# cyoq/onitama-alphazero

Hardware: AMD Instinct MI355X
Metric: MCTS node-expansions/sec/GPU @400 sims; self-play games/sec at 1/2/4/8 GPU (higher is better)
Workload: dtype fp32 (fp16x3 split)

## Files before the change

### onitama-alphazero_amd/csrc/oaz_engine.cpp

```cpp
#include <hip/hip_runtime.h>

#include <math.h>
#include <stddef.h>
#include <time.h>
#include <stdarg.h>
#include <stdio.h>
#include <stdlib.h>
#include <string.h>

#include <mutex>
#include <string>
#include <algorithm>
#include <vector>

#include "../../include/onitama_az.h"
#include "oaz_device.h"
#include "oaz_host.h"
#include "oaz_kernels.h"
#include "oaz_pack.h"
#include "oaz_weights_layout.h"

using namespace oaz;

static_assert(offsetof(oaz_config, search_time_ns) == 104 && offsetof(oaz_config, reuse_visits) == 116 &&
// ... 276 lines not shown
    if (!launch_reflect_samples) return oaz_set_err(OAZ_ERR_STATE, "reflect_samples: built without its kernel");
    RulesCtx* R = nullptr;
    std::unique_lock<std::mutex> lk;
    if (int rc = rules_begin(&R, lk)) return rc;
    hipStream_t st = R->stream;
    if (int rc = R->e.reserve(n)) return rc;
    if (int rc = R->f.reserve(n)) return rc;
    HIP_TRY(hipMemcpyAsync(R->e, in, n * sizeof(oaz_sample), hipMemcpyHostToDevice, st));
    HIP_TRY(launch_reflect_samples(R->e, n, R->f, st));
    HIP_TRY(hipMemcpyAsync(out, R->f, n * sizeof(oaz_sample), hipMemcpyDeviceToHost, st));
    HIP_TRY(hipStreamSynchronize(st));
    return 0;
}

constexpr int kMaxParts = 4;

enum LaunchKind { K_SELECT, K_NN, K_EXPAND, K_FINALIZE, K_NOISE, K_COMPACT, K_BACKUP_SELECT, K_COUNT };

struct TimedLaunch {
    LaunchKind kind;
    Event a, b;
    uint32_t samples;
};

struct LastSearch {
    uint32_t G = 0;
    uint32_t sims = 0;
    bool on_device = false;
    std::vector<uint32_t> per_game;
};
// ... 9 lines not shown
    uint32_t noise_chunk = 16;
    uint32_t G = 0, cap = 0, pathcap = 0, hcap = 0, out_cap = 0;
    int32_t sims_cap = 0;
    DevBuf<oaz_node> nodes;
    DevBuf<uint32_t> n_nodes, path, depth, leaf;
    DevBuf<oaz_state> leaf_state;
    DevBuf<uint64_t> stats, stats_sum;
    DevBuf<double> sqrt_tab;
    DevBuf<float> policy, value;
    DevBuf<uint8_t> need;
    DevBuf<uint32_t> slot, bcnt;
    DevBuf<oaz_state> cstate;
    DevBuf<float> weights;
    bool have_weights = false;
    DevBuf<unsigned long long> nn_fallback;
    DevBuf<oaz_state> s_roots;
    DevBuf<oaz_move> s_move;
    DevBuf<float> s_pi, s_rootv, s_rootp;
    uint32_t search_calls = 0;
    LastSearch last;
    DevBuf<uint64_t> deadline;
    DevBuf<uint32_t> sims_run;
    int wall_khz = 0;
    double t_search0 = 0.0;
    DevBuf<uint32_t> s_ply;
    DevBuf<oaz_state> root;
    DevBuf<uint32_t> ply, seq;
    DevBuf<uint64_t> game_id;
    DevBuf<uint8_t> active;
    DevBuf<oaz_sample> hist, out;
// ... 240 lines not shown
        for (auto& ev : e->ev_consumed[i])
            if (ev.create()) return OAZ_ERR_HIP;
    }
    if (hipDeviceGetAttribute(&e->cus, hipDeviceAttributeMultiprocessorCount, e->device) != hipSuccess || e->cus < 1)
        e->cus = 256;
    if (hipDeviceGetAttribute(&e->wall_khz, hipDeviceAttributeWallClockRate, e->device) != hipSuccess) e->wall_khz = 0;
    const size_t G = e->G;
    e->noise_chunk = noise_chunk_for(e);
    if (e->nodes.alloc(G * e->cap) || e->n_nodes.alloc(G) || e->path.alloc(G * e->pathcap) || e->depth.alloc(G) ||
        e->leaf.alloc(G) || e->leaf_state.alloc(G) || e->stats.alloc(G * GS_COUNT) || e->stats_sum.alloc(GS_COUNT) ||
        e->sqrt_tab.alloc((size_t)tree_visits_cap(cfg) + 2) || e->policy.alloc(G * 50) || e->value.alloc(G) || e->need.alloc(G) ||
        e->slot.alloc(G) || e->cstate.alloc(G + 16) || e->bcnt.alloc((size_t)buckets_of((uint32_t)G) + kMaxParts) ||
        e->weights.alloc(nn_device_floats(cfg->blocks, cfg->precision)) || e->s_roots.alloc(G) || e->s_move.alloc(G) ||
        e->s_pi.alloc(G * 50) || e->s_rootv.alloc(G) || e->s_rootp.alloc(G * 50) || e->s_ply.alloc(G) ||
        e->root.alloc(G) || e->ply.alloc(G) || e->seq.alloc(G) || e->game_id.alloc(G) || e->active.alloc(G) ||
        e->hist.alloc(G * e->hcap) || e->out.alloc(e->out_cap) || e->out_count.alloc(1) || e->nn_fallback.alloc(1) ||
        e->deadline.alloc(1) || e->sims_run.alloc(G) || e->fin.alloc(G) || e->fin_pos.alloc(G) ||
        (cfg->train_noise && e->noise.alloc(2 * (size_t)e->noise_chunk * G * kNoiseStride)))
        return OAZ_ERR_HIP;
    if (cfg->reuse_visits > 0 &&
        (e->adv_moves.alloc(G) || e->adv_codes.alloc(G) || e->adv_kept.alloc(G) || e->reuse_cnt.alloc(4)))
        return OAZ_ERR_HIP;
    if (cfg->temperature_plies > 0 && e->temp_cnt.alloc(2)) return OAZ_ERR_HIP;
    if (const size_t L = cfg->leaf_batch) {
        if (e->par_path.alloc(G * L * e->pathcap) || e->par_depth.alloc(G * L) || e->par_leaf.alloc(G * L) ||
            e->par_state.alloc(G * kMaxLeafBatch) || e->par_policy.alloc(G * kMaxLeafBatch * 50) ||
            e->par_value.alloc(G * kMaxLeafBatch) || e->par_stats.alloc(G * 3))
            return OAZ_ERR_HIP;
    }
    std::vector<double> tab((size_t)tree_visits_cap(cfg) + 2);
    for (size_t i = 0; i < tab.size(); ++i) tab[i] = sqrt((double)i);
    hipStream_t s0 = e->stream;
    HIP_TRY(hipMemcpyAsync(e->sqrt_tab, tab.data(), tab.size() * sizeof(double), hipMemcpyHostToDevice, s0));
    HIP_TRY(hipMemsetAsync(e->stats, 0, G * GS_COUNT * sizeof(uint64_t), s0));
    HIP_TRY(hipMemsetAsync(e->out_count, 0, sizeof(unsigned long long), s0));
    HIP_TRY(hipMemsetAsync(e->nn_fallback, 0, sizeof(unsigned long long), s0));
    HIP_TRY(hipMemsetAsync(e->active, 0, G, s0));
    HIP_TRY(hipMemsetAsync(e->need, 0, G, s0));
    HIP_TRY(hipMemsetAsync(e->slot, 0, G * sizeof(uint32_t), s0));
    HIP_TRY(hipMemsetAsync(e->cstate, 0, (G + 16) * sizeof(oaz_state), s0));
    if (e->reuse_cnt) HIP_TRY(hipMemsetAsync(e->reuse_cnt, 0, 4 * sizeof(uint64_t), s0));
    if (e->temp_cnt) HIP_TRY(hipMemsetAsync(e->temp_cnt, 0, 2 * sizeof(uint64_t), s0));
    if (e->par_state) {
        HIP_TRY(hipMemsetAsync(e->par_state, 0, G * kMaxLeafBatch * sizeof(oaz_state), s0));
        HIP_TRY(hipMemsetAsync(e->par_stats, 0, G * 3 * sizeof(uint64_t), s0));
    }
    HIP_TRY(hipStreamSynchronize(s0));
    if (cfg->evaluator == OAZ_EVAL_NN) {
        std::vector<float> w(oaz_weight_count(cfg->blocks, 64, 21));
        if (int rc = oaz_random_weights(0, cfg->blocks, w.data(), w.size())) return rc;
        if (int rc = oaz_load_weights(e, w.data(), w.size())) return rc;
// ... 135 lines not shown

extern "C" int oaz_kernel_times_get(oaz_engine* e, oaz_kernel_times* out) {
    if (!e || !out) return oaz_set_err(OAZ_ERR_ARG, "kernel_times: null");
    if (int rc = resolve_timing(e)) return rc;
    *out = e->times;
    return 0;
}

extern "C" int oaz_kernel_times_reset(oaz_engine* e) {
    if (!e) return oaz_set_err(OAZ_ERR_ARG, "kernel_times_reset: null");
    if (int rc = resolve_timing(e)) return rc;
    memset(&e->times, 0, sizeof(e->times));
    return 0;
}

static NNView nn_view(const oaz_engine* e, const TileMap* tm) {
    NNView w;
    w.blob = e->weights;
    w.blocks = e->cfg.blocks;
    w.precision = e->cfg.precision;
    w.x6_variant = 0;
#if OAZ_AB
    if (const char* xv = getenv("OAZ_NN_X6_V")) w.x6_variant = atoi(xv);
#endif
    w.blob_x6 = e->cfg.precision == OAZ_FP32_SPLIT16 ? e->weights + nn_packed_floats(e->cfg.blocks, OAZ_FP32_SPLIT16)
                                                     : nullptr;
    w.fallback = e->nn_fallback;
    w.tm = tm ? *tm : TileMap{nullptr, 0, 0};
    w.small_max = e->cus;
#if OAZ_AB
    if (const char* v = getenv("OAZ_NN_SMALL_MAX")) w.small_max = atoi(v);
#endif
    return w;
}

static int evaluate(oaz_engine* e, const oaz_state* d_states, uint32_t B, float* d_pol, float* d_val,
                    hipStream_t st = nullptr, const TileMap* tm = nullptr) {
    if (!st) st = e->stream;
    const uint32_t counted = tm ? 0u : B;
    if (e->cfg.evaluator == OAZ_EVAL_HASH)
        return timed(e, K_NN, counted, [&] { return launch_hash_eval(d_states, (int)B, d_pol, d_val, st); }, st);
    const NNView w = nn_view(e, tm);
    return timed(e, K_NN, counted, [&] { return launch_nn_forward(w, d_states, (int)B, d_pol, d_val, st); }, st);
}

extern "C" int oaz_nn_fallbacks(oaz_engine* e, uint64_t* tiles) {
    if (!e || !tiles) return oaz_set_err(OAZ_ERR_ARG, "nn_fallbacks: null");
    OAZ_ON_DEVICE(e->device);
    unsigned long long n = 0;
    HIP_TRY(hipMemcpyAsync(&n, e->nn_fallback, sizeof(n), hipMemcpyDeviceToHost, e->stream));
    HIP_TRY(hipStreamSynchronize(e->stream));
    *tiles = (uint64_t)n;
    return 0;
}

extern "C" int oaz_nn_forward(oaz_engine* e, const oaz_state* s, int B, float* policy, float* value) {
    if (!e || !s || B < 0) return oaz_set_err(OAZ_ERR_ARG, "nn_forward: bad arguments");
// ... 298 lines not shown
                if (int rc = backup(pc.fast)) return rc;
                for (int h = 0; h < P.n; ++h) P.part[h].active = pc.fullm + P.part[h].g0;
            }
            if (int rc = sim_step(e, S, P, ring, s, &spent)) return rc;
        }
        if (int rc = ring.release(c)) return rc;
    }
    if (int rc = backup(pc.fullm)) return rc;
    return P.join();
}

static int run_sims(oaz_engine* e, const TreeView& t, const oaz_state* roots, const uint8_t* active,
                    const uint64_t* gids, const uint32_t* plies, bool kept_trees = false, const PlyCap* pc = nullptr) {
    const bool budget = e->cfg.search_time_ns > 0, noise = e->cfg.train_noise && e->noise;
    const SearchPath path = pc ? PATH_STEPS : search_path(e, t.G, noise, kept_trees);
    const NNView w = nn_view(e, nullptr);
    Search S{t, roots, active, gids, plies, search_params(e), (uint32_t)e->cfg.sims, noise,
             e->cfg.evaluator == OAZ_EVAL_HASH ? nullptr : &w, budget ? e->deadline.get() : nullptr,
             budget ? e->sims_run.get() : nullptr};
    if (!pc && !compact_leaves(e, t.G)) {
        S.t.need = nullptr;
        S.t.slot = nullptr;
    }
    e->last = LastSearch{t.G};
    int rc = path == PATH_STEPS ? 0 : arm_device_budget(e, t.G);
    if (!rc)
        rc = pc                 ? run_capped(e, S, *pc)
             : path == PATH_PAR ? search_par(e, S)
             : path == PATH_LAT ? search_lat(e, S)
                                : run_chunks(e, S, path == PATH_GRP);
    if (rc) {
// ... 393 lines not shown
```

### onitama-alphazero_amd/csrc/oaz_kernels.h

```cpp
#pragma once

#include <hip/hip_runtime.h>
#include <stdint.h>

#include "../../include/onitama_az.h"
#include "oaz_device.h"
#include "oaz_nn_layout.h"

namespace oaz {

enum GameStat {
    GS_SIMS = 0,
    GS_EXPANSIONS,
    GS_CHILDREN,
    GS_TERMINAL,
    GS_DEPTH,
    GS_STUCK,
    GS_MAXNODES,
    GS_MOVES,
    GS_FINISHED,
    GS_CUT,
    GS_RED,
    GS_BLUE,
    GS_PASSES,
// ... 58 lines not shown
    const uint32_t* bcnt;
    int32_t nb;
    int32_t cap;
};
inline int32_t buckets_of(uint32_t G) { return (int32_t)((G + kBucket - 1) >> kBucketShift); }

struct NNView {
    const float* blob;
    int32_t blocks;
    int32_t precision;
    int32_t x6_variant;
    const float* blob_x6;
    unsigned long long* fallback;
    TileMap tm;
    int32_t small_max;
};

hipError_t launch_movegen(const oaz_state* s, int n, uint32_t* masks, oaz_move* moves,
                          uint8_t* counts, hipStream_t st);
hipError_t launch_step(oaz_state* s, const oaz_move* mv, int n, uint8_t* results, hipStream_t st);
hipError_t launch_current_state(const oaz_state* s, int n, uint8_t* results, hipStream_t st);
hipError_t launch_encode(const oaz_state* s, int n, float* planes, hipStream_t st);
__attribute__((weak)) hipError_t launch_reflect_samples(const oaz_sample* in, size_t n, oaz_sample* out, hipStream_t st);

hipError_t launch_nn_forward(const NNView& w, const oaz_state* s, int B, float* policy,
                             float* value, hipStream_t st);
hipError_t launch_hash_eval(const oaz_state* s, int B, float* policy, float* value, hipStream_t st);
hipError_t launch_eval_compact(const TreeView& t, hipStream_t st);

hipError_t launch_tree_reset(const TreeView& t, hipStream_t st);
constexpr int kNoiseStride = 2 * OAZ_MAX_MOVES;
hipError_t launch_select(const TreeView& t, const oaz_state* roots, const uint8_t* active,
                         const noise_t* noise , SearchParams p, hipStream_t st);
hipError_t launch_root_noise(const oaz_state* roots, const uint8_t* active, const uint64_t* game_id,
                             const uint32_t* ply, SearchParams p, uint32_t G, uint32_t sim0, uint32_t nsims,
                             noise_t* out , hipStream_t st);
hipError_t launch_expand_backup(const TreeView& t, const oaz_state* roots, const uint8_t* active,
                                const float* policy, const float* value, hipStream_t st);
hipError_t launch_backup_select(const TreeView& t, const oaz_state* roots, const uint8_t* active, const float* policy,
                                const float* value, const noise_t* noise, SearchParams p, hipStream_t st);
hipError_t launch_search_finalize(const TreeView& t, const oaz_state* roots, oaz_move* out_move,
// ... 45 lines not shown
```

### onitama-alphazero_amd/csrc/oaz_kernels.hip

```cpp
#include <hip/hip_runtime.h>
#include <stdlib.h>

#include <utility>

#include "oaz_device.h"
#include "oaz_kernels.h"

namespace oaz {

__constant__ AttackTable c_attack = make_attack_table();

constexpr int kWave = 64;
#ifndef OAZ_TREE_WPE
#define OAZ_TREE_WPE 8
#endif
#ifndef OAZ_TREE_WPB
#define OAZ_TREE_WPB 8
#endif
constexpr int kWavesPerBlock = OAZ_TREE_WPB;
constexpr int kBlock = kWave * kWavesPerBlock;

__device__ __forceinline__ int lane_id() { return (int)(threadIdx.x & 63); }
__device__ __forceinline__ uint32_t wave_game() {
    return blockIdx.x * kWavesPerBlock + (threadIdx.x >> 6);
// ... 621 lines not shown
    const int sl = seg_lane();
    constexpr uint32_t kB = (uint32_t)sizeof(noise_t);
    const __amdgpu_buffer_rsrc_t nr = __builtin_amdgcn_make_buffer_rsrc(
        (void*)noise, (short)0, (int)(t.G * (uint32_t)kNoiseStride * kB), 0x00020000);
#pragma unroll
    for (int c = C0; c < C1; ++c) {
        const int j = 16 * c + sl;
        const uint32_t off =
            go && j >= 1 && j < K ? (g * (uint32_t)kNoiseStride + 2u * (uint32_t)j) * kB : 0x80000000u;
        const auto d = __builtin_amdgcn_raw_buffer_load_b128(nr, (int)off, 0, 0);
        na[c] = __builtin_bit_cast(double, ((uint64_t)d[1] << 32) | d[0]);
        nb[c] = __builtin_bit_cast(double, ((uint64_t)d[3] << 32) | d[2]);
    }
}

constexpr int kWgGames = kWavesPerBlock * 4;
constexpr int kFoldRows = 32;
struct WgFold {
    int64_t kub[kFoldRows][kWgGames];
    double q[kFoldRows][kWgGames];
    double base[kFoldRows][kWgGames];
    double sq[kFoldRows][kWgGames];
    double nae[kFoldRows][kWgGames];
};
static_assert(sizeof(WgFold) <= 40960, "four workgroups' fold operands per CU");
struct FoldAcc {
    int K, acc;
    double qa, ba, sa;
};
__device__ __forceinline__ void wg_fold_pass(const WgFold* wf, const SearchParams& prm, FoldAcc& f, int pass) {
    const int gi = (int)threadIdx.x;
    const int off = pass ? kFoldRows : 0;
    const int j0 = pass ? kFoldRows : 1;
    const int jend = pass ? f.K : (f.K < kFoldRows ? f.K : kFoldRows);
    double nae = wf->nae[j0 - off][gi];
    int64_t kb = wf->kub[j0 - off][gi];
    for (int j = j0; __ballot(j < jend) != 0; ++j) {
        const int r = j - off, rn = r + 1 < kFoldRows ? r + 1 : kFoldRows - 1;
        const double qj = wf->q[r][gi], bj = wf->base[r][gi], sj = wf->sq[r][gi];
        const double nae_n = wf->nae[rn][gi];
        const int64_t kb_n = wf->kub[rn][gi];
        const double ua = f.qa + prm.c_puct * (f.ba + nae) * f.sa;
        const bool take = j < jend && !(total_key(ua) > kb);
        f.acc = take ? j : f.acc;
        f.qa = take ? qj : f.qa;
        f.ba = take ? bj : f.ba;
        f.sa = take ? sj : f.sa;
        nae = nae_n;
        kb = kb_n;
    }
}

template <class NA = NodesGlobal, bool WGF = false, bool WF_ALIASED = false>
__device__ __forceinline__ void select_seg_body(const TreeView& t, const oaz_state* __restrict__ roots,
                                                const uint8_t* __restrict__ active, const noise_t* __restrict__ noise,
                                                const SearchParams& prm, uint32_t g, oaz_state* leaf_lds = nullptr,
                                                const NA& na = NA{}, WgFold* wf = nullptr) {
    const int sl = seg_lane(), sb = seg_base();
    const bool on = g < t.G && !(active && active[g] != 1);
    const bool fold_mode = prm.train_noise && noise;
    oaz_node* T = t.nodes + (size_t)(on ? g : 0) * t.cap;
    const uint32_t pbase = (on ? g : 0u) * t.pathcap;
    uint32_t* const path = t.path;
    oaz_state s = load_state(na.root(roots, on ? g : 0));
    int color = s.to_move & 1;
    NodeRegs nd = load_node(na.at(T, 0));
    uint32_t node = 0, depth = 0;
    if (on && sl == 0) path[pbase] = 0;
    bool stuck = false;
    bool go = on && (node_flags(nd.misc) & 1) && !(node_flags(nd.misc) & 2);
    auto descend = [&](int best, const NodeRegs (&ch)[3]) {
        const int bc = best >> 4, src = sb + (best & 15);
// ... 44 lines not shown
            const int j = 16 * c + sl;
            if (go && j < K) {
                const FoldCh f = fold_chunk(ch[c], nza[c], nzb[c], sqn, prm);
                if (j != 0) wf->kub[j - r0][gi] = __builtin_bit_cast(int64_t, f.kub);
                wf->q[j - r0][gi] = f.q;
                wf->base[j - r0][gi] = f.base;
                wf->sq[j - r0][gi] = f.sq;
                wf->nae[j - r0][gi] = f.nae;
            }
        };
        stage(0, 0);
        stage(1, 0);
        if (sl == 0) wf->kub[0][gi] = go ? K : 0;
        __syncthreads();
        FoldAcc fa;
        if (threadIdx.x < (unsigned)kWgGames) {
            fa.K = (int)wf->kub[0][threadIdx.x];
            fa.acc = 0;
            fa.qa = wf->q[0][threadIdx.x];
            fa.ba = wf->base[0][threadIdx.x];
            fa.sa = wf->sq[0][threadIdx.x];
            wg_fold_pass(wf, prm, fa, 0);
            const bool more = __ballot(fa.K > kFoldRows) != 0;
            if (threadIdx.x == 0) wf->kub[kFoldRows - 1][0] = more ? 1 : 0;
        }
        __syncthreads();
        if (wf->kub[kFoldRows - 1][0] != 0) {
            root_noise_pairs<2, 3>(t, noise, g, go, K, nza, nzb);
            stage(2, kFoldRows);
            __syncthreads();
            if (threadIdx.x < (unsigned)kWgGames) wg_fold_pass(wf, prm, fa, 1);
            __syncthreads();
        }
        if (threadIdx.x < (unsigned)kWgGames) wf->kub[0][threadIdx.x] = fa.acc;
        __syncthreads();
        descend(go ? (int)wf->kub[0][gi] : 0, ch);
    }
    while (__builtin_amdgcn_read_exec() && __ballot(go)) {
        const int K = go ? node_nch(nd.misc) : 0;
        if (go && K == 0) {
            stuck = true;
            go = false;
        }
        NodeRegs ch[3];
        int64_t bkey = INT64_MIN;
        int bidx = sl;
#pragma unroll
        for (int c = 0; c < 3; ++c) {
            const int j = 16 * c + sl;
// ... 156 lines not shown
            }
        }
        ++depth;
        if (l == 0 && depth < t.pathcap) path[depth] = cidx;
        node = cidx;
        nd = c;
    }
    s.to_move = (uint8_t)color;
    w.node = node;
    w.depth = depth;
    w.stuck = stuck;
    w.nd = nd;
    w.dbg_cycles = dl;
}

__global__ void __launch_bounds__(kBlock) __attribute__((amdgpu_waves_per_eu(OAZ_TREE_WPE)))
k_select_seg(TreeView t, const oaz_state* __restrict__ roots, const uint8_t* __restrict__ active,
             const noise_t* __restrict__ noise, SearchParams prm) {
    __shared__ WgFold wf;
    select_seg_body<NodesGlobalRegs, true>(t, roots, active, noise, prm, seg_game(), nullptr, NodesGlobalRegs{}, &wf);
}

template <int N>
__device__ __forceinline__ float bcast_f32(float v) {
    return __int_as_float(__builtin_amdgcn_update_dpp(0, __float_as_int(v), 0x150 + N, 0xF, 0xF, false));
}
template <int SQ>
__device__ __forceinline__ void policy_sum_step(const float (&polm)[4], double& sum0, double& sum1) {
    constexpr int i0 = SQ, i1 = 25 + SQ;
    sum0 += (double)bcast_f32<(i0 & 15)>(polm[i0 >> 4]);
    sum1 += (double)bcast_f32<(i1 & 15)>(polm[i1 >> 4]);
}
template <int... SQ>
__device__ __forceinline__ void policy_sums(const float (&polm)[4], double& sum0, double& sum1,
                                            std::integer_sequence<int, SQ...>) {
// ... 130 lines not shown
        const double rk = ((depth - k) & 1) ? -r : r;
        oaz_node* np = na.at(T, n);
        np->N += 1;
        np->W += rk;
    }
}

__global__ void __launch_bounds__(kBlock) k_expand_backup_seg(TreeView t, const oaz_state* __restrict__ roots,
                                                              const uint8_t* __restrict__ active,
                                                              const float* __restrict__ policy,
                                                              const float* __restrict__ value) {
    __shared__ float spol[kWavesPerBlock * 4][52];
    expand_backup_seg_body(t, roots, active, policy, value, seg_game(), spol[threadIdx.x >> 4]);
}

__global__ void __launch_bounds__(kBlock) __attribute__((amdgpu_waves_per_eu(OAZ_TREE_WPE)))
k_backup_select_seg(TreeView t, const oaz_state* __restrict__ roots, const uint8_t* __restrict__ active,
                    const float* __restrict__ policy, const float* __restrict__ value, const noise_t* __restrict__ noise,
                    SearchParams prm) {
    union BackupSelectLds {
        float spol[kWavesPerBlock * 4][52];
        WgFold wf;
    };
    __shared__ BackupSelectLds lds;
    const uint32_t g = seg_game();
    expand_backup_seg_body(t, roots, active, policy, value, g, lds.spol[threadIdx.x >> 4], NodesGlobalRegs{});
    __builtin_amdgcn_fence(__ATOMIC_RELEASE, "workgroup");
    __builtin_amdgcn_fence(__ATOMIC_ACQUIRE, "workgroup");
    select_seg_body<NodesGlobalRegs, true, true>(t, roots, active, noise, prm, g, nullptr, NodesGlobalRegs{},
                                                 &lds.wf);
}

__device__ __forceinline__ void root_pi_best(const oaz_node* T, float* pi_out ,
                                             float& pi_lane, int& best_lane, int& K_out,
                                             uint32_t& best_mv) {
    const int l = lane_id();
    const NodeRegs root = load_node(&T[0]);
    const int K = (node_flags(root.misc) & 1) ? node_nch(root.misc) : 0;
    NodeRegs ch;
    ch.N = 0;
    ch.misc = 0;
    if (l < K) ch = load_node(&T[root.first + l]);
    const int bin = l < K ? (mv_slot(ch.misc) & 1) * 25 + mv_to(ch.misc) : -1;
    uint32_t cnt = 0;
    for (int j = 0; j < K; ++j) {
// ... 279 lines not shown
}
hipError_t launch_hash_eval(const oaz_state* s, int B, float* policy, float* value, hipStream_t st) {
    if (B <= 0) return hipSuccess;
    hipLaunchKernelGGL(k_hash_eval, dim3(thread_grid(B, 256)), dim3(256), 0, st, s, B, policy, value);
    return hipGetLastError();
}
hipError_t launch_eval_compact(const TreeView& t, hipStream_t st) {
    if (t.G == 0 || !t.need) return hipSuccess;
    hipLaunchKernelGGL(k_eval_compact, dim3((unsigned)buckets_of(t.G)), dim3(kCompactThreads), 0, st, t);
    return hipGetLastError();
}
hipError_t launch_tree_reset(const TreeView& t, hipStream_t st) {
    hipLaunchKernelGGL(k_tree_reset, dim3(thread_grid(t.G, kBlock)), dim3(kBlock), 0, st, t);
    return hipGetLastError();
}
static bool tree_seg() {
#if OAZ_AB
    static const bool v = !(getenv("OAZ_TREE_SEG") && getenv("OAZ_TREE_SEG")[0] == '0');
    return v;
#else
    return true;
#endif
}
bool tree_seg_kernels() { return tree_seg(); }
hipError_t launch_select(const TreeView& t, const oaz_state* roots, const uint8_t* active,
                         const noise_t* noise, SearchParams p, hipStream_t st) {
    if (tree_seg())
        hipLaunchKernelGGL(k_select_seg, dim3(wave_grid((t.G + 3) / 4)), dim3(kBlock), 0, st, t, roots, active, noise,
                           p);
    else
        hipLaunchKernelGGL(k_select, dim3(wave_grid(t.G)), dim3(kBlock), 0, st, t, roots, active, noise, p);
    return hipGetLastError();
}
hipError_t launch_root_noise(const oaz_state* roots, const uint8_t* active, const uint64_t* game_id,
                             const uint32_t* ply, SearchParams p, uint32_t G, uint32_t sim0, uint32_t nsims,
                             noise_t* out, hipStream_t st) {
    hipLaunchKernelGGL(k_root_noise, dim3(wave_grid(G)), dim3(kBlock), 0, st, roots, active, game_id, ply, p, G,
                       sim0, nsims, out);
    return hipGetLastError();
}
hipError_t launch_expand_backup(const TreeView& t, const oaz_state* roots, const uint8_t* active,
                                const float* policy, const float* value, hipStream_t st) {
    if (tree_seg())
        hipLaunchKernelGGL(k_expand_backup_seg, dim3(wave_grid((t.G + 3) / 4)), dim3(kBlock), 0, st, t, roots, active,
                           policy, value);
    else
        hipLaunchKernelGGL(k_expand_backup, dim3(wave_grid(t.G)), dim3(kBlock), 0, st, t, roots, active, policy,
                           value);
    return hipGetLastError();
}
hipError_t launch_backup_select(const TreeView& t, const oaz_state* roots, const uint8_t* active, const float* policy,
                                const float* value, const noise_t* noise, SearchParams p, hipStream_t st) {
    if (!tree_seg()) {
        if (hipError_t err = launch_expand_backup(t, roots, active, policy, value, st)) return err;
        return launch_select(t, roots, active, noise, p, st);
    }
    hipLaunchKernelGGL(k_backup_select_seg, dim3(wave_grid((t.G + 3) / 4)), dim3(kBlock), 0, st, t, roots, active,
                       policy, value, noise, p);
    return hipGetLastError();
}
hipError_t launch_search_finalize(const TreeView& t, const oaz_state* roots, oaz_move* out_move,
                                  float* out_pi, hipStream_t st) {
    hipLaunchKernelGGL(k_search_finalize, dim3(wave_grid(t.G)), dim3(kBlock), 0, st, t, roots,
                       out_move, out_pi);
    return hipGetLastError();
}
hipError_t launch_selfplay_move(const TreeView& t, const SlotView& s, hipStream_t st) {
    hipLaunchKernelGGL(k_selfplay_move, dim3(wave_grid(t.G)), dim3(kBlock), 0, st, t, s);
    hipLaunchKernelGGL(k_samples_scan, dim3(1), dim3(kScanThreads), 0, st, s);
    hipLaunchKernelGGL(k_samples_emit, dim3(wave_grid(t.G)), dim3(kBlock), 0, st, t, s);
    return hipGetLastError();
}
// ... 28 lines not shown
```

### onitama-alphazero_amd/csrc/oaz_nn.hip

```cpp
#include <hip/hip_runtime.h>

#include <utility>

#include "oaz_device.h"
#include "oaz_kernels.h"

namespace oaz {

typedef float f32x4 __attribute__((ext_vector_type(4)));
typedef __bf16 bf16x8 __attribute__((ext_vector_type(8)));

namespace nn {
constexpr int kCh = 64;
constexpr int kSB = 16;
constexpr int kWaves = 8;
constexpr int kTPW = 13;
constexpr int kRS = 72;
constexpr int kScratch = 128;
constexpr int kLdsFloats = kSB * 25 * kRS + kWaves * kScratch;
}

struct TileSpan {
    int b0, end, cap;
};
// ... 499 lines not shown
        }
    return P;
}
template <int GRP, int KH>
struct ConvPlanOf {
    static constexpr ConvPlan P = conv_plan(GRP, KH);
};

struct X6Cfg {
    static constexpr int WAVES = 8, KH = OAZ_H3_KH, NS = 15, GRP0 = 3, GRP1 = 4;
};
template <int BF_, int DBG_ = 0>
struct H3Cfg {
    static constexpr int kSplit = BF_ ? kH1Split : kH3Split;
    static constexpr int WAVES = 8, KH = OAZ_H3_KH, NS = kSplit > 12 ? kSplit : 25 - kSplit, GRP0 = BF_ ? 9 : 7,
                         GRP1 = BF_ ? 10 : 8, BF = BF_, DBG = DBG_;
};

template <int GRP, int KH, int K, int N>
__device__ __forceinline__ void x6_load(bf16x8 (&a)[N], const char* img, const int (&ab)[2][3], int piece) {
    constexpr ConvBatch B = ConvPlanOf<GRP, KH>::P.b[K];
#pragma unroll
    for (int q = 0; q < N; ++q)
        if (q < B.n) {
            const int off = B.nb[q] * (nn::kSB * x6::kRowB) + piece * 128;
            a[q] = *reinterpret_cast<const bf16x8*>(img + ab[B.m][off >> 16] + (off & 0xffff));
        }
}

template <int GRP, int KH, int K, int NS, int N>
__device__ __forceinline__ void x6_mfma(f32x4 (&acc)[NS], const bf16x8 (&a)[N], const bf16x8& bv) {
// ... 394 lines not shown
        b[1] = b[0];
    } else {
        b[0] = h3_ldb(W, ((B0.t * 2 + B0.m) * 2 + 0) * 4);
        b[1] = h3_ldb(W, ((B0.t * 2 + B0.m) * 2 + 1) * 4);
    }
}

template <class C, int GRP, int... K>
__device__ __forceinline__ void conv_h3_run(f32x4 (&acc)[C::NS], const char* img, const FragW& W, const int (&lo)[2],
                                            const f16x8 (&bfirst)[2], std::integer_sequence<int, K...>) {
    int ab[2][2];
#pragma unroll
    for (int m = 0; m < 2; ++m)
#pragma unroll
        for (int sg = 0; sg < 2; ++sg) ab[m][sg] = lo[m] + sg * 65536;
    f16x8 b[2] = {bfirst[0], bfirst[1]}, bn[2];
    if constexpr (!h3_pf<C>()) h3_first_b<C, GRP>(b, W);
    if constexpr (C::BF) {
        f16x8 X[C::KH], X2[C::KH];
        h3_load<C, GRP, 0>(X, img, ab, 0);
        ((K % 2 == 0 ? conv_h1_batch<C, GRP, K>(acc, img, W, b, bn, X, X2, ab)
                     : conv_h1_batch<C, GRP, K>(acc, img, W, b, bn, X2, X, ab)),
         ...);
    } else {
        f16x8 X[C::KH], Y[C::KH];
        h3_load<C, GRP, 0>(X, img, ab, 1);
        (conv_h3_batch<C, GRP, K>(acc, img, W, b, bn, X, Y, ab), ...);
    }
}

// ... 336 lines not shown
    h3_heads<C>(p, img, lo, wave, lane, b0, B, policy, value);
    if constexpr (C::DBG == 2) {
        stamp(5);
        __syncthreads();
        float v = 0.0f;
#pragma unroll
        for (int k = 0; k < 8; ++k) v = lane == k ? (float)ph[k] : v;
        if (lane < 8 && b0 + nn::kSB <= B) policy[(size_t)b0 * 50 + wave * 8 + lane] = v;
    }
    if constexpr (C::BF) return false;
    return h3_overflowed(hmax);
}

template <class C>
struct H3Fallback {
    static constexpr bool kOn = !C::BF && C::DBG == 0;
    using X = X6Cfg;
    static constexpr int kBase = h3::kLdsFloats + h3::kLutB / 4;
    static constexpr int kLds = kOn && x6::kLdsFloats > kBase ? x6::kLdsFloats : kBase;
};

template <class X, int GRP>
__device__ __noinline__ void nn_h3_fallback(const oaz_state* __restrict__ states, const TileSpan sp,
                                            const float* __restrict__ xblob,
                                            int blocks, float* __restrict__ policy, float* __restrict__ value,
                                            float* lds) {
    nn_x6_body<X, GRP>(states, sp, xblob, blocks, policy, value, lds);
}
template <class C>
__device__ __forceinline__ void nn_h3_recompute(const oaz_state* states, const TileSpan sp, const float* xblob,
                                                int blocks, float* policy, float* value, float* lds,
                                                unsigned long long* fallback) {
    using X = typename H3Fallback<C>::X;
    if ((threadIdx.x >> 8) == 0)
        nn_h3_fallback<X, X::GRP0>(states, sp, xblob, blocks, policy, value, lds);
    else
        nn_h3_fallback<X, X::GRP1>(states, sp, xblob, blocks, policy, value, lds);
    if (threadIdx.x == 0) atomicAdd(fallback, 1ull);
}

template <class C, class States>
__device__ __forceinline__ void nn_h3_tile(const States& states, const TileSpan sp, const float* blob, int blocks,
                                           const float* xblob, unsigned long long* fallback, float* policy,
                                           float* value, float* lds, int opaque = 0) {
    bool ovf;
    if ((threadIdx.x >> 8) == 0) {
        __builtin_amdgcn_s_setprio(1);
        ovf = nn_h3_body<C, C::GRP0>(states, sp, blob, blocks, policy, value, lds, opaque);
    } else {
        ovf = nn_h3_body<C, C::GRP1>(states, sp, blob, blocks, policy, value, lds, opaque);
    }
    if constexpr (H3Fallback<C>::kOn) {
        if (__syncthreads_or(ovf)) nn_h3_recompute<C>(states, sp, xblob, blocks, policy, value, lds, fallback);
    }
}

template <class C>
__global__ void __launch_bounds__(64 * C::WAVES) k_nn_h3(const oaz_state* __restrict__ states, int B,
                                                        const float* __restrict__ blob, int blocks,
                                                        float* __restrict__ policy, float* __restrict__ value,
                                                        const float* __restrict__ xblob,
                                                        unsigned long long* __restrict__ fallback, TileMap tm) {
    __shared__ __attribute__((aligned(16))) float lds[H3Fallback<C>::kLds];
    const uint64_t rt0 = C::DBG == 5 ? __builtin_amdgcn_s_memrealtime() : 0;
    const TileSpan sp = tile_span(tm, B);
    nn_h3_tile<C>(states, sp, blob, blocks, xblob, fallback, policy, value, lds);
    if constexpr (C::DBG == 5) {
        __syncthreads();
        if (threadIdx.x == 0 && sp.b0 < sp.end) {
            const uint64_t rt1 = __builtin_amdgcn_s_memrealtime();
            const uint32_t hw = __builtin_amdgcn_s_getreg((31 << 11) | 4);
            const uint32_t xcc = __builtin_amdgcn_s_getreg((15 << 11) | 20);
            uint32_t* o = reinterpret_cast<uint32_t*>(policy + (size_t)sp.b0 * 50);
            o[0] = (uint32_t)rt0;
            o[1] = (uint32_t)(rt0 >> 32);
            o[2] = (uint32_t)rt1;
            o[3] = (uint32_t)(rt1 >> 32);
            o[4] = hw;
            o[5] = xcc;
        }
    }
}

namespace h3s {
constexpr int kRows = 26;
constexpr int kZero = 25;
constexpr int kRowB = 128;
constexpr int kPlaneB = kRows * kRowB;
constexpr int kImageB = 2 * kPlaneB;
constexpr int kSkipOff = 2 * kImageB;
constexpr int kHeadOff = kSkipOff + 4 * 64 * 2 * 16;
constexpr int kHeadF = (int)nnl::kHeadsLen<OAZ_FP32_SPLIT16>;
constexpr int kFeatOff = kHeadOff + ((kHeadF * 4 + 15) & ~15);
constexpr int kBytes = kFeatOff + (16 * 80 + 16 * 128) * 4;
__device__ __forceinline__ int chunk_off(int row, int c8) { return row * kRowB + ((c8 ^ (row & 7)) << 4); }
// ... 320 lines not shown
    int b = (int)blockIdx.x, end = B, cap = B;
    if (tm.bcnt) {
        const int bk = (int)blockIdx.x % tm.nb;
        b = (bk << kBucketShift) + (int)blockIdx.x / tm.nb;
        end = (bk << kBucketShift) + (int)tm.bcnt[bk];
        cap = tm.cap;
    }
    if (b >= end) return;
    const bool ovf = nn_h3s_body<C>(states, b, blob, blocks, policy, value, lds);
    if constexpr (H3Fallback<C>::kOn) {
        if (__syncthreads_or(ovf))
            nn_h3_recompute<C>(states, TileSpan{b, b + 1, cap}, xblob, blocks, policy, value, lds, fallback);
    }
}

hipError_t launch_nn_forward(const NNView& w, const oaz_state* s, int B, float* policy, float* value,
                             hipStream_t st) {
    if (B <= 0) return hipSuccess;
    const int per_bucket = ((B < (int)kBucket ? B : (int)kBucket) + nn::kSB - 1) / nn::kSB;
    const unsigned grid = w.tm.bcnt ? (unsigned)(w.tm.nb * per_bucket) : (unsigned)((B + nn::kSB - 1) / nn::kSB);
    const dim3 block(64 * nn::kWaves);
    if (w.precision == OAZ_FP32_SPLIT16) {
        if (!w.fallback || !w.blob_x6) return hipErrorInvalidValue;
        if (B <= w.small_max) {
            const unsigned g1 = w.tm.bcnt ? (unsigned)(w.tm.nb * (B < (int)kBucket ? B : (int)kBucket)) : (unsigned)B;
            auto ks = k_nn_h3s<H3Cfg<0>>;
#if OAZ_AB
            if (w.x6_variant == 70) ks = k_nn_h3s<H3Cfg<0, 2>>;
#endif
            hipLaunchKernelGGL(ks, dim3(g1), block, 0, st, s, B, w.blob, w.blocks, policy, value,
                               w.blob_x6, w.fallback, w.tm);
            return hipGetLastError();
        }
        auto k = k_nn_h3<H3Cfg<0>>;
#if OAZ_AB
        switch (w.x6_variant) {
            case 36: k = k_nn_h3<H3Cfg<0, 2>>; break;
            case 40: k = k_nn_h3<H3Cfg<0, 3>>; break;
            case 41: k = k_nn_h3<H3Cfg<0, 4>>; break;
            case 47: k = k_nn_h3<H3Cfg<0, 7>>; break;
            case 49: k = k_nn_h3<H3Cfg<0, 9>>; break;
            case 60: k = k_nn_h3<H3Cfg<0, 5>>; break;
            default: break;
        }
#endif
        hipLaunchKernelGGL(k, dim3(grid), block, 0, st, s, B, w.blob, w.blocks, policy, value, w.blob_x6, w.fallback,
                           w.tm);
    } else if (w.precision == OAZ_FP32_SPLIT) {
        hipLaunchKernelGGL(k_nn_x6<X6Cfg>, dim3(grid), block, 0, st, s, B, w.blob, w.blocks, policy, value, w.tm);
    } else if (w.precision == OAZ_BF16) {
        hipLaunchKernelGGL(k_nn_h3<H3Cfg<1>>, dim3(grid), block, 0, st, s, B, w.blob, w.blocks, policy, value, nullptr,
                           nullptr, w.tm);
    } else {
        hipLaunchKernelGGL(k_nn_sq16, dim3(grid), block, 0, st, s, B, w.blob, w.blocks, policy, value, w.tm);
    }
    return hipGetLastError();
}

}
```

Measured before the change: 51.50 million.

## Defer NN overflow recompute to a redo kernel and shrink tree workgroups to four waves

```diff
diff --git a/onitama-alphazero_amd/csrc/oaz_engine.cpp b/onitama-alphazero_amd/csrc/oaz_engine.cpp
--- a/onitama-alphazero_amd/csrc/oaz_engine.cpp
+++ b/onitama-alphazero_amd/csrc/oaz_engine.cpp
@@ -314,6 +314,7 @@
 }
 
 constexpr int kMaxParts = 4;
+static size_t redo_lists_words(uint32_t G) { return (size_t)kMaxParts * redo_words(redo_tiles(G)); }
 
 enum LaunchKind { K_SELECT, K_NN, K_EXPAND, K_FINALIZE, K_NOISE, K_COMPACT, K_BACKUP_SELECT, K_COUNT };
 
@@ -353,6 +354,7 @@
     DevBuf<float> weights;
     bool have_weights = false;
     DevBuf<unsigned long long> nn_fallback;
+    uint32_t* nn_redo = nullptr;
     DevBuf<oaz_state> s_roots;
     DevBuf<oaz_move> s_move;
     DevBuf<float> s_pi, s_rootv, s_rootp;
@@ -623,7 +625,8 @@
         e->weights.alloc(nn_device_floats(cfg->blocks, cfg->precision)) || e->s_roots.alloc(G) || e->s_move.alloc(G) ||
         e->s_pi.alloc(G * 50) || e->s_rootv.alloc(G) || e->s_rootp.alloc(G * 50) || e->s_ply.alloc(G) ||
         e->root.alloc(G) || e->ply.alloc(G) || e->seq.alloc(G) || e->game_id.alloc(G) || e->active.alloc(G) ||
-        e->hist.alloc(G * e->hcap) || e->out.alloc(e->out_cap) || e->out_count.alloc(1) || e->nn_fallback.alloc(1) ||
+        e->hist.alloc(G * e->hcap) || e->out.alloc(e->out_cap) || e->out_count.alloc(1) ||
+        e->nn_fallback.alloc(2 + (cfg->precision == OAZ_FP32_SPLIT16 ? redo_lists_words((uint32_t)G) / 2 + 1 : 0)) ||
         e->deadline.alloc(1) || e->sims_run.alloc(G) || e->fin.alloc(G) || e->fin_pos.alloc(G) ||
         (cfg->train_noise && e->noise.alloc(2 * (size_t)e->noise_chunk * G * kNoiseStride)))
         return OAZ_ERR_HIP;
@@ -644,6 +647,11 @@
     HIP_TRY(hipMemsetAsync(e->stats, 0, G * GS_COUNT * sizeof(uint64_t), s0));
     HIP_TRY(hipMemsetAsync(e->out_count, 0, sizeof(unsigned long long), s0));
     HIP_TRY(hipMemsetAsync(e->nn_fallback, 0, sizeof(unsigned long long), s0));
+    if (cfg->precision == OAZ_FP32_SPLIT16 && launch_nn_redo_clear) {
+        uint32_t* lists = reinterpret_cast<uint32_t*>(e->nn_fallback.get() + 2);
+        HIP_TRY(launch_nn_redo_clear(lists, redo_lists_words((uint32_t)G), s0));
+        e->nn_redo = lists;
+    }
     HIP_TRY(hipMemsetAsync(e->active, 0, G, s0));
     HIP_TRY(hipMemsetAsync(e->need, 0, G, s0));
     HIP_TRY(hipMemsetAsync(e->slot, 0, G * sizeof(uint32_t), s0));
@@ -809,8 +817,13 @@
     return 0;
 }
 
-static NNView nn_view(const oaz_engine* e, const TileMap* tm) {
+static NNView nn_view(const oaz_engine* e, const TileMap* tm, hipStream_t st) {
     NNView w;
+    w.redo = nullptr;
+    w.redo_cap = redo_tiles(e->G);
+    for (int h = 0; e->nn_redo && h < kMaxParts; ++h)
+        if (st == (h ? (hipStream_t)e->stream3[h - 1] : (hipStream_t)e->stream))
+            w.redo = e->nn_redo + (size_t)h * redo_words(w.redo_cap);
     w.blob = e->weights;
     w.blocks = e->cfg.blocks;
     w.precision = e->cfg.precision;
@@ -835,7 +848,7 @@
     const uint32_t counted = tm ? 0u : B;
     if (e->cfg.evaluator == OAZ_EVAL_HASH)
         return timed(e, K_NN, counted, [&] { return launch_hash_eval(d_states, (int)B, d_pol, d_val, st); }, st);
-    const NNView w = nn_view(e, tm);
+    const NNView w = nn_view(e, tm, st);
     return timed(e, K_NN, counted, [&] { return launch_nn_forward(w, d_states, (int)B, d_pol, d_val, st); }, st);
 }
 
@@ -1164,7 +1177,7 @@
                     const uint64_t* gids, const uint32_t* plies, bool kept_trees = false, const PlyCap* pc = nullptr) {
     const bool budget = e->cfg.search_time_ns > 0, noise = e->cfg.train_noise && e->noise;
     const SearchPath path = pc ? PATH_STEPS : search_path(e, t.G, noise, kept_trees);
-    const NNView w = nn_view(e, nullptr);
+    const NNView w = nn_view(e, nullptr, e->stream);
     Search S{t, roots, active, gids, plies, search_params(e), (uint32_t)e->cfg.sims, noise,
              e->cfg.evaluator == OAZ_EVAL_HASH ? nullptr : &w, budget ? e->deadline.get() : nullptr,
              budget ? e->sims_run.get() : nullptr};
diff --git a/onitama-alphazero_amd/csrc/oaz_kernels.h b/onitama-alphazero_amd/csrc/oaz_kernels.h
--- a/onitama-alphazero_amd/csrc/oaz_kernels.h
+++ b/onitama-alphazero_amd/csrc/oaz_kernels.h
@@ -96,7 +96,13 @@
     unsigned long long* fallback;
     TileMap tm;
     int32_t small_max;
+    uint32_t* redo;
+    uint32_t redo_cap;
 };
+constexpr int kRedoCount = 0, kRedoDone = 1, kRedoSpans = 4;
+constexpr unsigned kRedoGrid = 4;
+inline size_t redo_words(uint32_t tiles) { return (size_t)kRedoSpans + 5 * (size_t)tiles; }
+inline uint32_t redo_tiles(uint32_t G) { return (G + 15) / 16 + 256 * (uint32_t)buckets_of(G); }
 
 hipError_t launch_movegen(const oaz_state* s, int n, uint32_t* masks, oaz_move* moves,
                           uint8_t* counts, hipStream_t st);
@@ -107,6 +113,7 @@
 
 hipError_t launch_nn_forward(const NNView& w, const oaz_state* s, int B, float* policy,
                              float* value, hipStream_t st);
+__attribute__((weak)) hipError_t launch_nn_redo_clear(uint32_t* redo, size_t words, hipStream_t st);
 hipError_t launch_hash_eval(const oaz_state* s, int B, float* policy, float* value, hipStream_t st);
 hipError_t launch_eval_compact(const TreeView& t, hipStream_t st);
 
diff --git a/onitama-alphazero_amd/csrc/oaz_kernels.hip b/onitama-alphazero_amd/csrc/oaz_kernels.hip
--- a/onitama-alphazero_amd/csrc/oaz_kernels.hip
+++ b/onitama-alphazero_amd/csrc/oaz_kernels.hip
@@ -659,21 +659,27 @@
     }
 }
 
-constexpr int kWgGames = kWavesPerBlock * 4;
 constexpr int kFoldRows = 32;
-struct WgFold {
-    int64_t kub[kFoldRows][kWgGames];
-    double q[kFoldRows][kWgGames];
-    double base[kFoldRows][kWgGames];
-    double sq[kFoldRows][kWgGames];
-    double nae[kFoldRows][kWgGames];
+template <int WPB>
+struct WgFoldT {
+    static constexpr int kGames = WPB * 4;
+    int64_t kub[kFoldRows][kGames];
+    double q[kFoldRows][kGames];
+    double base[kFoldRows][kGames];
+    double sq[kFoldRows][kGames];
+    double nae[kFoldRows][kGames];
 };
+using WgFold = WgFoldT<kWavesPerBlock>;
+constexpr int kStepWaves = 4;
+using WgFold4 = WgFoldT<kStepWaves>;
 static_assert(sizeof(WgFold) <= 40960, "four workgroups' fold operands per CU");
+static_assert(sizeof(WgFold4) <= 20480, "a 4-wave workgroup's fold operands: two beside a k_nn_h3 workgroup, eight per CU");
 struct FoldAcc {
     int K, acc;
     double qa, ba, sa;
 };
-__device__ __forceinline__ void wg_fold_pass(const WgFold* wf, const SearchParams& prm, FoldAcc& f, int pass) {
+template <class WF>
+__device__ __forceinline__ void wg_fold_pass(const WF* wf, const SearchParams& prm, FoldAcc& f, int pass) {
     const int gi = (int)threadIdx.x;
     const int off = pass ? kFoldRows : 0;
     const int j0 = pass ? kFoldRows : 1;
@@ -696,11 +702,11 @@
     }
 }
 
-template <class NA = NodesGlobal, bool WGF = false, bool WF_ALIASED = false>
+template <class NA = NodesGlobal, bool WGF = false, bool WF_ALIASED = false, class WF = WgFold>
 __device__ __forceinline__ void select_seg_body(const TreeView& t, const oaz_state* __restrict__ roots,
                                                 const uint8_t* __restrict__ active, const noise_t* __restrict__ noise,
                                                 const SearchParams& prm, uint32_t g, oaz_state* leaf_lds = nullptr,
-                                                const NA& na = NA{}, WgFold* wf = nullptr) {
+                                                const NA& na = NA{}, WF* wf = nullptr) {
     const int sl = seg_lane(), sb = seg_base();
     const bool on = g < t.G && !(active && active[g] != 1);
     const bool fold_mode = prm.train_noise && noise;
@@ -775,7 +781,7 @@
         if (sl == 0) wf->kub[0][gi] = go ? K : 0;
         __syncthreads();
         FoldAcc fa;
-        if (threadIdx.x < (unsigned)kWgGames) {
+        if (threadIdx.x < (unsigned)WF::kGames) {
             fa.K = (int)wf->kub[0][threadIdx.x];
             fa.acc = 0;
             fa.qa = wf->q[0][threadIdx.x];
@@ -790,10 +796,10 @@
             root_noise_pairs<2, 3>(t, noise, g, go, K, nza, nzb);
             stage(2, kFoldRows);
             __syncthreads();
-            if (threadIdx.x < (unsigned)kWgGames) wg_fold_pass(wf, prm, fa, 1);
+            if (threadIdx.x < (unsigned)WF::kGames) wg_fold_pass(wf, prm, fa, 1);
             __syncthreads();
         }
-        if (threadIdx.x < (unsigned)kWgGames) wf->kub[0][threadIdx.x] = fa.acc;
+        if (threadIdx.x < (unsigned)WF::kGames) wf->kub[0][threadIdx.x] = fa.acc;
         __syncthreads();
         descend(go ? (int)wf->kub[0][gi] : 0, ch);
     }
@@ -980,11 +986,21 @@
     w.dbg_cycles = dl;
 }
 
+#if OAZ_AB
 __global__ void __launch_bounds__(kBlock) __attribute__((amdgpu_waves_per_eu(OAZ_TREE_WPE)))
 k_select_seg(TreeView t, const oaz_state* __restrict__ roots, const uint8_t* __restrict__ active,
              const noise_t* __restrict__ noise, SearchParams prm) {
     __shared__ WgFold wf;
     select_seg_body<NodesGlobalRegs, true>(t, roots, active, noise, prm, seg_game(), nullptr, NodesGlobalRegs{}, &wf);
+}
+#endif
+__device__ __forceinline__ uint32_t seg_game4() { return blockIdx.x * (kStepWaves * 4) + (threadIdx.x >> 4); }
+__global__ void __launch_bounds__(kWave * kStepWaves) __attribute__((amdgpu_waves_per_eu(OAZ_TREE_WPE)))
+k_select_seg4(TreeView t, const oaz_state* __restrict__ roots, const uint8_t* __restrict__ active,
+              const noise_t* __restrict__ noise, SearchParams prm) {
+    __shared__ WgFold4 wf;
+    select_seg_body<NodesGlobalRegs, true, false, WgFold4>(t, roots, active, noise, prm, seg_game4(), nullptr,
+                                                           NodesGlobalRegs{}, &wf);
 }
 
 template <int N>
@@ -1145,6 +1161,7 @@
     expand_backup_seg_body(t, roots, active, policy, value, seg_game(), spol[threadIdx.x >> 4]);
 }
 
+#if OAZ_AB
 __global__ void __launch_bounds__(kBlock) __attribute__((amdgpu_waves_per_eu(OAZ_TREE_WPE)))
 k_backup_select_seg(TreeView t, const oaz_state* __restrict__ roots, const uint8_t* __restrict__ active,
                     const float* __restrict__ policy, const float* __restrict__ value, const noise_t* __restrict__ noise,
@@ -1160,6 +1177,24 @@
     __builtin_amdgcn_fence(__ATOMIC_ACQUIRE, "workgroup");
     select_seg_body<NodesGlobalRegs, true, true>(t, roots, active, noise, prm, g, nullptr, NodesGlobalRegs{},
                                                  &lds.wf);
+}
+#endif
+__global__ void __launch_bounds__(kWave * kStepWaves) __attribute__((amdgpu_waves_per_eu(OAZ_TREE_WPE)))
+k_backup_select_seg4(TreeView t, const oaz_state* __restrict__ roots, const uint8_t* __restrict__ active,
+                     const float* __restrict__ policy, const float* __restrict__ value,
+                     const noise_t* __restrict__ noise, SearchParams prm) {
+    union BackupSelectLds {
+        float spol[kStepWaves * 4][52];
+        WgFold4 wf;
+    };
+    __shared__ BackupSelectLds lds;
+    static_assert(sizeof(BackupSelectLds) <= 20480, "two 4-wave tree workgroups beside a k_nn_h3 workgroup");
+    const uint32_t g = seg_game4();
+    expand_backup_seg_body(t, roots, active, policy, value, g, lds.spol[threadIdx.x >> 4], NodesGlobalRegs{});
+    __builtin_amdgcn_fence(__ATOMIC_RELEASE, "workgroup");
+    __builtin_amdgcn_fence(__ATOMIC_ACQUIRE, "workgroup");
+    select_seg_body<NodesGlobalRegs, true, true, WgFold4>(t, roots, active, noise, prm, g, nullptr, NodesGlobalRegs{},
+                                                          &lds.wf);
 }
 
 __device__ __forceinline__ void root_pi_best(const oaz_node* T, float* pi_out ,
@@ -1469,6 +1504,7 @@
     hipLaunchKernelGGL(k_tree_reset, dim3(thread_grid(t.G, kBlock)), dim3(kBlock), 0, st, t);
     return hipGetLastError();
 }
+static inline unsigned step_grid(uint32_t G) { return (G + kStepWaves * 4 - 1) / (kStepWaves * 4); }
 static bool tree_seg() {
 #if OAZ_AB
     static const bool v = !(getenv("OAZ_TREE_SEG") && getenv("OAZ_TREE_SEG")[0] == '0');
@@ -1478,11 +1514,24 @@
 #endif
 }
 bool tree_seg_kernels() { return tree_seg(); }
+#if OAZ_AB
+static bool step_waves8() {
+    static const bool v = getenv("OAZ_STEP_WAVES") && getenv("OAZ_STEP_WAVES")[0] == '8';
+    return v;
+}
+#endif
 hipError_t launch_select(const TreeView& t, const oaz_state* roots, const uint8_t* active,
                          const noise_t* noise, SearchParams p, hipStream_t st) {
-    if (tree_seg())
+#if OAZ_AB
+    if (tree_seg() && step_waves8()) {
         hipLaunchKernelGGL(k_select_seg, dim3(wave_grid((t.G + 3) / 4)), dim3(kBlock), 0, st, t, roots, active, noise,
                            p);
+        return hipGetLastError();
+    }
+#endif
+    if (tree_seg())
+        hipLaunchKernelGGL(k_select_seg4, dim3(step_grid(t.G)), dim3(kWave * kStepWaves), 0, st, t, roots, active,
+                           noise, p);
     else
         hipLaunchKernelGGL(k_select, dim3(wave_grid(t.G)), dim3(kBlock), 0, st, t, roots, active, noise, p);
     return hipGetLastError();
@@ -1510,7 +1559,14 @@
         if (hipError_t err = launch_expand_backup(t, roots, active, policy, value, st)) return err;
         return launch_select(t, roots, active, noise, p, st);
     }
-    hipLaunchKernelGGL(k_backup_select_seg, dim3(wave_grid((t.G + 3) / 4)), dim3(kBlock), 0, st, t, roots, active,
+#if OAZ_AB
+    if (step_waves8()) {
+        hipLaunchKernelGGL(k_backup_select_seg, dim3(wave_grid((t.G + 3) / 4)), dim3(kBlock), 0, st, t, roots, active,
+                           policy, value, noise, p);
+        return hipGetLastError();
+    }
+#endif
+    hipLaunchKernelGGL(k_backup_select_seg4, dim3(step_grid(t.G)), dim3(kWave * kStepWaves), 0, st, t, roots, active,
                        policy, value, noise, p);
     return hipGetLastError();
 }
diff --git a/onitama-alphazero_amd/csrc/oaz_nn.hip b/onitama-alphazero_amd/csrc/oaz_nn.hip
--- a/onitama-alphazero_amd/csrc/oaz_nn.hip
+++ b/onitama-alphazero_amd/csrc/oaz_nn.hip
@@ -537,7 +537,13 @@
 struct H3Cfg {
     static constexpr int kSplit = BF_ ? kH1Split : kH3Split;
     static constexpr int WAVES = 8, KH = OAZ_H3_KH, NS = kSplit > 12 ? kSplit : 25 - kSplit, GRP0 = BF_ ? 9 : 7,
-                         GRP1 = BF_ ? 10 : 8, BF = BF_, DBG = DBG_;
+                         GRP1 = BF_ ? 10 : 8, BF = BF_, DBG = DBG_, LIST = 0;
+};
+template <int DBG_ = 0>
+struct H3ListCfg {
+    static constexpr int kSplit = kH1Split;
+    static constexpr int WAVES = 8, KH = OAZ_H3_KH, NS = kSplit > 12 ? kSplit : 25 - kSplit, GRP0 = 9, GRP1 = 10, BF = 0,
+                         DBG = DBG_, LIST = 1;
 };
 
 template <int GRP, int KH, int K, int N>
@@ -962,6 +968,7 @@
     for (int m = 0; m < 2; ++m)
 #pragma unroll
         for (int sg = 0; sg < 2; ++sg) ab[m][sg] = lo[m] + sg * 65536;
+    if constexpr (C::LIST) asm("" : "+v"(ab[0][1]), "+v"(ab[1][1]));
     f16x8 b[2] = {bfirst[0], bfirst[1]}, bn[2];
     if constexpr (!h3_pf<C>()) h3_first_b<C, GRP>(b, W);
     if constexpr (C::BF) {
@@ -1328,7 +1335,7 @@
 
 template <class C>
 struct H3Fallback {
-    static constexpr bool kOn = !C::BF && C::DBG == 0;
+    static constexpr bool kOn = !C::BF && C::DBG == 0 && !C::LIST;
     using X = X6Cfg;
     static constexpr int kBase = h3::kLdsFloats + h3::kLutB / 4;
     static constexpr int kLds = kOn && x6::kLdsFloats > kBase ? x6::kLdsFloats : kBase;
@@ -1356,7 +1363,8 @@
 template <class C, class States>
 __device__ __forceinline__ void nn_h3_tile(const States& states, const TileSpan sp, const float* blob, int blocks,
                                            const float* xblob, unsigned long long* fallback, float* policy,
-                                           float* value, float* lds, int opaque = 0) {
+                                           float* value, float* lds, int opaque = 0, uint32_t* redo = nullptr,
+                                           uint32_t redo_cap = 0) {
     bool ovf;
     if ((threadIdx.x >> 8) == 0) {
         __builtin_amdgcn_s_setprio(1);
@@ -1364,7 +1372,19 @@
     } else {
         ovf = nn_h3_body<C, C::GRP1>(states, sp, blob, blocks, policy, value, lds, opaque);
     }
-    if constexpr (H3Fallback<C>::kOn) {
+    if constexpr (C::LIST && !C::BF && C::DBG == 0) {
+        if (__ballot(ovf) != 0 && (threadIdx.x & 63) == 0 && blockIdx.x < redo_cap &&
+            atomicExch(&redo[kRedoSpans + 4 * (size_t)redo_cap + blockIdx.x], 1u) == 0u) {
+            const uint32_t k = atomicAdd(&redo[kRedoCount], 1u);
+            if (k < redo_cap) {
+                int* e = reinterpret_cast<int*>(redo + kRedoSpans) + 4 * (size_t)k;
+                e[0] = sp.b0;
+                e[1] = sp.end;
+                e[2] = sp.cap;
+                e[3] = (int)blockIdx.x;
+            }
+        }
+    } else if constexpr (H3Fallback<C>::kOn) {
         if (__syncthreads_or(ovf)) nn_h3_recompute<C>(states, sp, xblob, blocks, policy, value, lds, fallback);
     }
 }
@@ -1374,11 +1394,13 @@
                                                         const float* __restrict__ blob, int blocks,
                                                         float* __restrict__ policy, float* __restrict__ value,
                                                         const float* __restrict__ xblob,
-                                                        unsigned long long* __restrict__ fallback, TileMap tm) {
+                                                        unsigned long long* __restrict__ fallback, TileMap tm,
+                                                        uint32_t* __restrict__ redo, uint32_t redo_cap) {
     __shared__ __attribute__((aligned(16))) float lds[H3Fallback<C>::kLds];
+    static_assert(!C::LIST || sizeof(lds) <= 110592, "k_nn_h3: 110,592 B of LDS leave a tree workgroup 53 KB of the CU's");
     const uint64_t rt0 = C::DBG == 5 ? __builtin_amdgcn_s_memrealtime() : 0;
     const TileSpan sp = tile_span(tm, B);
-    nn_h3_tile<C>(states, sp, blob, blocks, xblob, fallback, policy, value, lds);
+    nn_h3_tile<C>(states, sp, blob, blocks, xblob, fallback, policy, value, lds, 0, redo, redo_cap);
     if constexpr (C::DBG == 5) {
         __syncthreads();
         if (threadIdx.x == 0 && sp.b0 < sp.end) {
@@ -1393,6 +1415,36 @@
             o[4] = hw;
             o[5] = xcc;
         }
+    }
+}
+
+template <class X>
+__global__ void __launch_bounds__(64 * X::WAVES) k_nn_h3_redo(const oaz_state* __restrict__ states,
+                                                             const float* __restrict__ xblob, int blocks,
+                                                             float* __restrict__ policy, float* __restrict__ value,
+                                                             unsigned long long* __restrict__ fallback,
+                                                             uint32_t* __restrict__ redo, uint32_t redo_cap) {
+    __shared__ __attribute__((aligned(16))) float lds[x6::kLdsFloats];
+    const uint32_t cnt = redo[kRedoCount];
+    if (cnt == 0) return;
+    const uint32_t n = cnt < redo_cap ? cnt : redo_cap;
+    const int* spans = reinterpret_cast<const int*>(redo + kRedoSpans);
+    for (uint32_t k = blockIdx.x; k < n; k += gridDim.x) {
+        const TileSpan sp{spans[4 * (size_t)k], spans[4 * (size_t)k + 1], spans[4 * (size_t)k + 2]};
+        const uint32_t tile = (uint32_t)spans[4 * (size_t)k + 3];
+        if ((threadIdx.x >> 8) == 0)
+            nn_x6_body<X, X::GRP0>(states, sp, xblob, blocks, policy, value, lds);
+        else
+            nn_x6_body<X, X::GRP1>(states, sp, xblob, blocks, policy, value, lds);
+        if (threadIdx.x == 0) {
+            atomicAdd(fallback, 1ull);
+            if (tile < redo_cap) atomicExch(&redo[kRedoSpans + 4 * (size_t)redo_cap + tile], 0u);
+        }
+        __syncthreads();
+    }
+    if (threadIdx.x == 0 && atomicAdd(&redo[kRedoDone], 1u) == gridDim.x - 1) {
+        atomicExch(&redo[kRedoDone], 0u);
+        atomicExch(&redo[kRedoCount], 0u);
     }
 }
 
@@ -1743,6 +1795,16 @@
     }
 }
 
+__global__ void __launch_bounds__(256) k_nn_redo_clear(uint32_t* redo, size_t words) {
+    for (size_t i = (size_t)blockIdx.x * 256 + threadIdx.x; i < words; i += (size_t)gridDim.x * 256) redo[i] = 0u;
+}
+hipError_t launch_nn_redo_clear(uint32_t* redo, size_t words, hipStream_t st) {
+    if (words == 0) return hipSuccess;
+    const size_t blocks = (words + 255) / 256;
+    hipLaunchKernelGGL(k_nn_redo_clear, dim3((unsigned)(blocks < 1024 ? blocks : 1024)), dim3(256), 0, st, redo, words);
+    return hipGetLastError();
+}
+
 hipError_t launch_nn_forward(const NNView& w, const oaz_state* s, int B, float* policy, float* value,
                              hipStream_t st) {
     if (B <= 0) return hipSuccess;
@@ -1761,25 +1823,29 @@
                                w.blob_x6, w.fallback, w.tm);
             return hipGetLastError();
         }
-        auto k = k_nn_h3<H3Cfg<0>>;
+        if (!w.redo || grid > w.redo_cap) return hipErrorInvalidValue;
+        auto k = k_nn_h3<H3ListCfg<0>>;
 #if OAZ_AB
         switch (w.x6_variant) {
-            case 36: k = k_nn_h3<H3Cfg<0, 2>>; break;
-            case 40: k = k_nn_h3<H3Cfg<0, 3>>; break;
-            case 41: k = k_nn_h3<H3Cfg<0, 4>>; break;
-            case 47: k = k_nn_h3<H3Cfg<0, 7>>; break;
-            case 49: k = k_nn_h3<H3Cfg<0, 9>>; break;
-            case 60: k = k_nn_h3<H3Cfg<0, 5>>; break;
+            case 36: k = k_nn_h3<H3ListCfg<2>>; break;
+            case 40: k = k_nn_h3<H3ListCfg<3>>; break;
+            case 41: k = k_nn_h3<H3ListCfg<4>>; break;
+            case 47: k = k_nn_h3<H3ListCfg<7>>; break;
+            case 49: k = k_nn_h3<H3ListCfg<9>>; break;
+            case 60: k = k_nn_h3<H3ListCfg<5>>; break;
             default: break;
         }
 #endif
         hipLaunchKernelGGL(k, dim3(grid), block, 0, st, s, B, w.blob, w.blocks, policy, value, w.blob_x6, w.fallback,
-                           w.tm);
+                           w.tm, w.redo, w.redo_cap);
+        if (hipError_t err = hipGetLastError()) return err;
+        hipLaunchKernelGGL(k_nn_h3_redo<X6Cfg>, dim3(grid < kRedoGrid ? grid : kRedoGrid), block, 0, st, s, w.blob_x6,
+                           w.blocks, policy, value, w.fallback, w.redo, w.redo_cap);
     } else if (w.precision == OAZ_FP32_SPLIT) {
         hipLaunchKernelGGL(k_nn_x6<X6Cfg>, dim3(grid), block, 0, st, s, B, w.blob, w.blocks, policy, value, w.tm);
     } else if (w.precision == OAZ_BF16) {
         hipLaunchKernelGGL(k_nn_h3<H3Cfg<1>>, dim3(grid), block, 0, st, s, B, w.blob, w.blocks, policy, value, nullptr,
-                           nullptr, w.tm);
+                           nullptr, w.tm, nullptr, 0u);
     } else {
         hipLaunchKernelGGL(k_nn_sq16, dim3(grid), block, 0, st, s, B, w.blob, w.blocks, policy, value, w.tm);
     }
```

Result: no change. 51.04 million (-0.9%).
